# zju3dv/pats

Hardware: AMD Instinct MI355X
Metric: image-pairs/sec (coarse+fine OT) on 640x480 MegaDepth; OT iters/sec per pair (higher is better)
Workload: dtype f32 (contractions: fp32 operands split into fp16 hi + lo, three exact-product MFMA passes, fp32 accumulate)

## Files before the change

include/pats_amd.h:

```cpp
#ifndef PATS_AMD_H
#define PATS_AMD_H

#include <stddef.h>
#include <stdint.h>

#ifdef __cplusplus
extern "C" {
#endif

typedef void* pats_stream_t;

enum {
    PATS_OK = 0,
    PATS_ERR_INVALID = 1,
    PATS_ERR_UNSUPPORTED = 2,
    PATS_ERR_LAUNCH = 3,
    PATS_ERR_NO_DEVICE = 4
};

enum { PATS_SINKHORN_AUTO = 0, PATS_SINKHORN_LOG = 1, PATS_SINKHORN_KERNEL = 2 };

const char* pats_version(void);
#define PATS_ABI_VERSION 8
int pats_abi_version(void);
const char* pats_last_error(void);
int pats_device_count(void);
int pats_set_sinkhorn_mode(int mode);
int pats_set_fine_fused(int on);

int pats_sinkhorn_fallbacks(int64_t* count, int reset);

int pats_cost_f32(const float* d0, const float* d1, int64_t batch, int D, int n, int m, float* out,
                  pats_stream_t stream);

size_t pats_sinkhorn_workspace_bytes(int64_t batch, int M, int N);
int pats_sinkhorn_f32(const float* Z, int64_t batch, int M, int N, const float* log_mu,
                      const float* log_nu, int iters, float* out, void* workspace,
                      size_t workspace_bytes, pats_stream_t stream);

size_t pats_ot_workspace_bytes(int64_t batch, int M, int N);
int pats_log_optimal_transport_f32(const float* scores, int64_t batch, int m, int n,
                                   const float* alpha, const float* ns, int iters, float* Z,
                                   void* workspace, size_t workspace_bytes, pats_stream_t stream);

size_t pats_ot2_workspace_bytes(int64_t batch, int m, int n);
int pats_log_optimal_transport2_flags_f32(const float* scores, int64_t batch, int m, int n,
                                          const float* one, const float* ns, int iters, float bias_k,
                                          float* Z, uint8_t* col_nomatch, void* workspace,
                                          size_t workspace_bytes, pats_stream_t stream);
int pats_log_optimal_transport2_f32(const float* scores, int64_t batch, int m, int n,
                                    const float* one, const float* ns, int iters, float bias_k,
                                    float* Z, void* workspace, size_t workspace_bytes,
                                    pats_stream_t stream);

int pats_cost_ot_f32(const float* d0, const float* d1, int64_t batch, int D, int n, int m,
                     int variant, const float* scalar, const float* ns, int iters, float bias_k,
                     float* Z, void* workspace, size_t workspace_bytes, pats_stream_t stream);
size_t pats_cost_ot_workspace_bytes(int64_t batch, int D, int n, int m, int variant);
int pats_cost_ot_flags_f32(const float* d0, const float* d1, int64_t batch, int D, int n, int m,
                           int variant, const float* scalar, const float* ns, int iters, float bias_k,
                           float* Z, uint8_t* col_nomatch, void* workspace, size_t workspace_bytes,
                           pats_stream_t stream);

int pats_set_cost_ot_mid_event(void* event);

int pats_cost_ot_flags_counted_f32(const float* d0, const float* d1, int64_t batch_cap, const int64_t* batch_dev,
                                   int D, int n, int m, int variant, const float* scalar, const float* ns, int iters,
                                   float bias_k, float* Z, uint8_t* col_nomatch, void* workspace,
                                   size_t workspace_bytes, pats_stream_t stream);

int pats_colmass_sqrt_f32(const float* Z, int64_t batch, int M, int N, float* out,
                          pats_stream_t stream);
int pats_colmass_flags_f32(const float* Z, int64_t batch, int M, int N, float* out, uint8_t* col_nomatch,
                           pats_stream_t stream);
int pats_dustbin_bias_inplace_f32(float* Z, int64_t batch, int M, int N, float k,
                                  pats_stream_t stream);
int pats_exp_f32(const float* Z, int64_t count, float* out, pats_stream_t stream);

int pats_argmax_f32(const float* Z, int64_t batch, int M, int N, int64_t* row_arg,
                    int64_t* col_arg, pats_stream_t stream);

int pats_iterative_expand_f32(const float* P, int input_is_log, int64_t batch, int M, int N,
                              const float* scalex, const float* scaley, int lim3, int h, int w,
                              float lower_bound, int iter_num, float* whole_cost, float* core_cost,
                              float* average_point, float* x_scale, float* y_scale, int64_t* bound,
                              uint8_t* row_nomatch, pats_stream_t stream);

int pats_iterative_expand_counted_f32(const float* P, int input_is_log, int64_t batch_cap, const int64_t* batch_dev,
                                      int M, int N, const float* scalex, const float* scaley, int lim3, int h, int w,
                                      float lower_bound, int iter_num, float* whole_cost, float* core_cost,
                                      float* average_point, float* x_scale, float* y_scale, int64_t* bound,
                                      uint8_t* row_nomatch, pats_stream_t stream);

int pats_split_patches(const int32_t* sum_cycle_host, int height, int width, int max_once_used,
                       int64_t* second_layer_set, int64_t* third_layer_set);
int pats_split_patches_device(const int32_t* sum_cycle, int64_t pairs, int height, int width,
                              int max_once_used, int64_t* second_layer_set, int64_t* third_layer_set,
                              int32_t* cycle_num, pats_stream_t stream);

int pats_compute_imgs_bounds_f32(const float* x_scale, const float* y_scale,
                                 const float* average_point, const uint8_t* if_nomatching, int Np,
                                 int height, int width, int img, int64_t* bound5, int64_t* K_out,
                                 float* x_scale_new, float* y_scale_new, float* average_new,
                                 pats_stream_t stream);

int pats_left_crops_f32(const float* left, int n_img, int H, int W, const int64_t* bound5, int64_t K,
                        int height, int width, float* out, pats_stream_t stream);

int pats_compute_imgs_bounds_batch_f32(const float* x_scale, const float* y_scale, const float* average_point,
                                       const uint8_t* if_nomatching, int n_img, int Np, int height, int width,
                                       int64_t* bound5, int64_t* K_img, int64_t* K_total, float* x_scale_new,
// ... 266 lines not shown
```

pats_amd/_lib.py:

```python
import ctypes
import os

_HERE = os.path.dirname(os.path.abspath(__file__))
LIB_PATH = os.path.join(_HERE, "libpats_amd.so")
if os.environ.get("PATS_AMD_DIAG_LIB", "") not in ("", "0"):
    _sfx = os.environ["PATS_AMD_DIAG_LIB"]
    LIB_PATH = os.path.join(_HERE, "libpats_amd_diag%s.so" % ("" if _sfx == "1" else _sfx))

c_void_p, c_int, c_i64, c_f, c_size = (ctypes.c_void_p, ctypes.c_int, ctypes.c_int64, ctypes.c_float,
                                       ctypes.c_size_t)

ABI_VERSION = 8



class PairTable(ctypes.Structure):
    _fields_ = [("pairs", ctypes.c_int64), ("shape_host", c_void_p), ("cell_base_host", c_void_p), ("shape", c_void_p),
                ("cell_base", c_void_p), ("img_base", c_void_p)]


_TAB = ctypes.POINTER(PairTable)


class CropFormat(ctypes.Structure):
    _fields_ = [("dtype", ctypes.c_int32), ("layout", ctypes.c_int32), ("normalize", ctypes.c_int32),
                ("mean", ctypes.c_float * 3), ("std", ctypes.c_float * 3)]


_FMT = ctypes.POINTER(CropFormat)

SIGNATURES = {
    "pats_version": (ctypes.c_char_p, []),
    "pats_abi_version": (c_int, []),
    "pats_last_error": (ctypes.c_char_p, []),
    "pats_device_count": (c_int, []),
    "pats_set_sinkhorn_mode": (c_int, [c_int]),
    "pats_set_fine_fused": (c_int, [c_int]),
    "pats_sinkhorn_fallbacks": (c_int, [ctypes.POINTER(ctypes.c_int64), c_int]),
    "pats_set_gnn_redo_mode": (c_int, [c_int]),
    "pats_gnn_overflows": (c_int, [ctypes.POINTER(ctypes.c_int64), c_int]),
    "pats_cost_f32": (c_int, [c_void_p, c_void_p, c_i64, c_int, c_int, c_int, c_void_p, c_void_p]),
    "pats_sinkhorn_workspace_bytes": (c_size, [c_i64, c_int, c_int]),
    "pats_sinkhorn_f32": (c_int, [c_void_p, c_i64, c_int, c_int, c_void_p, c_void_p, c_int, c_void_p,
                                  c_void_p, c_size, c_void_p]),
    "pats_ot_workspace_bytes": (c_size, [c_i64, c_int, c_int]),
    "pats_log_optimal_transport_f32": (c_int, [c_void_p, c_i64, c_int, c_int, c_void_p, c_void_p, c_int,
                                               c_void_p, c_void_p, c_size, c_void_p]),
    "pats_ot2_workspace_bytes": (c_size, [c_i64, c_int, c_int]),
    "pats_log_optimal_transport2_f32": (c_int, [c_void_p, c_i64, c_int, c_int, c_void_p, c_void_p, c_int,
                                                c_f, c_void_p, c_void_p, c_size, c_void_p]),
    "pats_cost_ot_f32": (c_int, [c_void_p, c_void_p, c_i64, c_int, c_int, c_int, c_int, c_void_p,
                                 c_void_p, c_int, c_f, c_void_p, c_void_p, c_size, c_void_p]),
    "pats_cost_ot_flags_f32": (c_int, [c_void_p, c_void_p, c_i64, c_int, c_int, c_int, c_int, c_void_p,
                                       c_void_p, c_int, c_f, c_void_p, c_void_p, c_void_p, c_size, c_void_p]),
    "pats_set_cost_ot_mid_event": (c_int, [c_void_p]),
    "pats_cost_ot_flags_counted_f32": (c_int, [c_void_p, c_void_p, c_i64, c_void_p, c_int, c_int, c_int, c_int, c_void_p,
                                               c_void_p, c_int, c_f, c_void_p, c_void_p, c_void_p, c_size, c_void_p]),
    "pats_iterative_expand_counted_f32": (c_int, [c_void_p, c_int, c_i64, c_void_p, c_int, c_int, c_void_p, c_void_p, c_int,
                                                  c_int, c_int, c_f, c_int, c_void_p, c_void_p, c_void_p,
                                                  c_void_p, c_void_p, c_void_p, c_void_p, c_void_p]),
    "pats_fine_descriptors_counted_f32": (c_int, [c_void_p, c_void_p, c_void_p, c_void_p, c_void_p, c_i64, c_void_p, c_int,
                                                  c_void_p, c_void_p]),
    "pats_log_optimal_transport2_flags_f32": (c_int, [c_void_p, c_i64, c_int, c_int, c_void_p, c_void_p, c_int,
                                                      c_f, c_void_p, c_void_p, c_void_p, c_size, c_void_p]),
    "pats_colmass_flags_f32": (c_int, [c_void_p, c_i64, c_int, c_int, c_void_p, c_void_p, c_void_p]),
    "pats_cost_ot_workspace_bytes": (c_size, [c_i64, c_int, c_int, c_int, c_int]),
    "pats_colmass_sqrt_f32": (c_int, [c_void_p, c_i64, c_int, c_int, c_void_p, c_void_p]),
    "pats_dustbin_bias_inplace_f32": (c_int, [c_void_p, c_i64, c_int, c_int, c_f, c_void_p]),
    "pats_exp_f32": (c_int, [c_void_p, c_i64, c_void_p, c_void_p]),
    "pats_argmax_f32": (c_int, [c_void_p, c_i64, c_int, c_int, c_void_p, c_void_p, c_void_p]),
    "pats_iterative_expand_f32": (c_int, [c_void_p, c_int, c_i64, c_int, c_int, c_void_p, c_void_p, c_int,
                                          c_int, c_int, c_f, c_int, c_void_p, c_void_p, c_void_p,
                                          c_void_p, c_void_p, c_void_p, c_void_p, c_void_p]),
    "pats_split_patches": (c_int, [c_void_p, c_int, c_int, c_int, c_void_p, c_void_p]),
    "pats_split_patches_device": (c_int, [c_void_p, c_i64, c_int, c_int, c_int, c_void_p, c_void_p, c_void_p, c_void_p]),
    "pats_compute_imgs_bounds_batch_f32": (c_int, [c_void_p, c_void_p, c_void_p, c_void_p, c_int, c_int, c_int, c_int,
                                                   c_void_p, c_void_p, c_void_p, c_void_p, c_void_p, c_void_p, c_void_p]),
    "pats_left_crops_counted_f32": (c_int, [c_void_p, c_int, c_int, c_int, c_void_p, c_i64, c_void_p, c_int, c_int,
                                            c_void_p, c_void_p]),
    "pats_tensor_resize_hwc_counted_f32": (c_int, [c_void_p, c_int, c_int, c_int, c_int, c_void_p, c_i64, c_void_p,
                                                   c_void_p, c_void_p, c_void_p]),
    "pats_compute_imgs_bounds_f32": (c_int, [c_void_p, c_void_p, c_void_p, c_void_p, c_int, c_int, c_int,
                                             c_int, c_void_p, c_void_p, c_void_p, c_void_p, c_void_p,
                                             c_void_p]),
    "pats_left_crops_f32": (c_int, [c_void_p, c_int, c_int, c_int, c_void_p, c_i64, c_int, c_int, c_void_p,
                                    c_void_p]),
    "pats_tensor_resize_f32": (c_int, [c_void_p, c_int, c_int, c_int, c_int, c_void_p, c_i64, c_void_p,
                                       c_void_p, c_void_p]),
    "pats_tensor_resize_hwc_f32": (c_int, [c_void_p, c_int, c_int, c_int, c_int, c_void_p, c_i64,
                                           c_void_p, c_void_p, c_void_p]),
    "pats_compute_result_f32": (c_int, [c_void_p, c_int, c_i64, c_void_p, c_void_p, c_void_p, c_void_p,
                                        c_int, c_void_p, c_void_p, c_void_p, c_void_p, c_void_p,
                                        c_void_p]),
    "pats_compute_result_ws_f32": (c_int, [c_void_p, c_int, c_i64, c_void_p, c_void_p, c_void_p, c_void_p,
                                           c_int, c_void_p, c_void_p, c_void_p, c_void_p, c_void_p,
                                           c_void_p, c_size, c_void_p]),
    "pats_fine_descriptors_f32": (c_int, [c_void_p, c_void_p, c_void_p, c_void_p, c_void_p, c_i64, c_void_p, c_void_p]),
    "pats_third_descriptors_f32": (c_int, [c_void_p, c_void_p, c_void_p, c_void_p, c_void_p, c_void_p, c_void_p,
                                           c_i64, c_i64, c_void_p, c_void_p, c_void_p, c_void_p, c_void_p]),
    "pats_third_level_f32": (c_int, [c_void_p, c_void_p, c_i64, c_int, c_void_p, c_void_p, c_void_p, c_void_p,
                                     c_void_p, c_int, c_int, c_void_p, c_void_p, c_void_p, c_void_p, c_void_p,
                                     c_void_p]),
    "pats_third_descriptors_counted_f32": (c_int, [c_void_p, c_void_p, c_void_p, c_void_p, c_void_p, c_void_p, c_void_p,
                                                   c_i64, c_void_p, c_i64, c_void_p, c_void_p, c_void_p, c_void_p, c_void_p]),
    "pats_fine_descriptors_nhwc_f32": (c_int, [c_void_p, c_void_p, c_void_p, c_void_p, c_void_p, c_i64, c_void_p, c_void_p]),
    "pats_third_descriptors_nhwc_f32": (c_int, [c_void_p, c_void_p, c_void_p, c_void_p, c_void_p, c_void_p, c_void_p,
                                                c_i64, c_void_p, c_i64, c_void_p, c_void_p, c_void_p, c_void_p, c_void_p]),
    "pats_fine_descriptors_typed": (c_int, [c_void_p, c_void_p, c_void_p, c_int, c_int, c_void_p, c_void_p, c_i64, c_void_p,
                                            c_void_p, c_void_p]),
    "pats_third_descriptors_typed": (c_int, [c_void_p, c_void_p, c_int, c_int, c_void_p, c_void_p, c_void_p, c_void_p, c_void_p,
                                             c_i64, c_void_p, c_i64, c_void_p, c_void_p, c_void_p, c_void_p, c_void_p]),
    "pats_third_level_counted_f32": (c_int, [c_void_p, c_void_p, c_i64, c_void_p, c_int, c_void_p, c_void_p, c_void_p,
                                             c_void_p, c_void_p, c_int, c_int, c_void_p, c_void_p, c_void_p, c_void_p,
                                             c_void_p]),
    "pats_chunk_rows_workspace_bytes": (c_size, [c_i64, c_int]),
    "pats_chunk_rows_device": (c_int, [c_void_p, c_i64, c_int, c_int, c_int, c_int, c_i64] + [c_void_p] * 13 +
                               [c_size, c_void_p]),
    "pats_profile_marker": (c_int, [c_int, c_void_p]),
    "pats_stream_create_cu_mask": (c_int, [c_void_p, c_int, c_void_p]),
    "pats_stream_destroy": (c_int, [c_void_p]),
# ... 106 lines not shown
```

pats_amd/csrc/gather.hip:

```cpp
#include "common.hpp"

#include <cstdlib>

namespace pats {

template <int POL, typename T>
__device__ __forceinline__ T ldm(const T* p) {
    if (POL & 1) return __builtin_nontemporal_load(p);
    return *p;
}
template <int POL, typename T>
__device__ __forceinline__ void stm(T* p, T v) {
    if (POL & 2) __builtin_nontemporal_store(v, p);
    else *p = v;
}

typedef float f2u __attribute__((ext_vector_type(2), aligned(4)));
template <int POL>
__device__ __forceinline__ f2u ldm2(const float* p) {
    const f2u* q = reinterpret_cast<const f2u*>(p);
    if (POL & 1) return __builtin_nontemporal_load(q);
    return *q;
}

template <int POL>
__global__ void __launch_bounds__(256)
fine_desc_kernel(const float* __restrict__ f0, const float* __restrict__ f1,
                 const float* __restrict__ f2, const float* __restrict__ title,
                 const float* __restrict__ rubbish, int64_t B, float* __restrict__ desc,
                 const int64_t* __restrict__ B_live) {
    const int64_t n = blockIdx.x;
    const int64_t b = n % B;
    if (B_live && b >= *B_live) return;
    const int lane = threadIdx.x & 63, wave = threadIdx.x >> 6;
    float* o = desc + n * 264 * 145;
    int pt[3], off0[3], off1[3];
    bool live[3];
#pragma unroll
    for (int g = 0; g < 3; ++g) {
        const int p = lane + 64 * g;
        live[g] = p < 145;
        pt[g] = p < 144 ? p : 0;
        const int r = pt[g] / 12, c = pt[g] - r * 12;
        off0[g] = (4 * r + 1) * 48 + 4 * c + 1;
        off1[g] = (2 * r) * 24 + 2 * c;
    }
    const bool dust = lane == 16;
    auto put = [&](int ch, float v0, float v1, float v2) {
        float* row = o + ch * 145;
        stm<POL>(row + lane, v0);
        stm<POL>(row + lane + 64, v1);
        if (live[2]) stm<POL>(row + lane + 128, dust ? rubbish[b * 264 + ch] : v2);
    };
    for (int ch = wave; ch < 8; ch += 4) {
        const float v = title[b * 8 + ch];
        put(ch, v, v, v);
    }
#pragma unroll 2
    for (int ch = 8 + wave; ch < 72; ch += 4) {
        const float* m = f0 + (n * 64 + (ch - 8)) * 48 * 48;
        float v[3];
#pragma unroll
        for (int g = 0; g < 3; ++g) {
            const float* q = m + off0[g];
            const f2u a = ldm2<POL>(q), c2 = ldm2<POL>(q + 48);
            v[g] = (((a.x + a.y) + c2.x) + c2.y) / 4.0f;
        }
        put(ch, v[0], v[1], v[2]);
    }
#pragma unroll 2
    for (int ch = 72 + wave; ch < 136; ch += 4) {
        const float* m = f1 + (n * 64 + (ch - 72)) * 24 * 24;
        float v[3];
#pragma unroll
        for (int g = 0; g < 3; ++g) {
            const float* q = m + off1[g];
            const f2u a = ldm2<POL>(q), c2 = ldm2<POL>(q + 24);
            v[g] = (((a.x + a.y) + c2.x) + c2.y) / 4.0f;
        }
        put(ch, v[0], v[1], v[2]);
    }
#pragma unroll 4
    for (int ch = 136 + wave; ch < 264; ch += 4) {
        const float* m = f2 + (n * 128 + (ch - 136)) * 144;
        put(ch, ldm<POL>(m + pt[0]), ldm<POL>(m + pt[1]), ldm<POL>(m + pt[2]));
    }
}

__device__ __forceinline__ long long round_half_even_div(float x, float d) {
    return (long long)rintf(x / d);
}

template <int POL>
__global__ void __launch_bounds__(256)
third_desc_kernel(const float* __restrict__ ff0, const float* __restrict__ ff1,
                  const float* __restrict__ mk0, const float* __restrict__ mk1,
                  const int64_t* __restrict__ b_ids, const float* __restrict__ kenc,
                  const float* __restrict__ rubbish, int64_t P, int64_t B,
                  float* __restrict__ out0, float* __restrict__ out1, int64_t* __restrict__ ps_out,
                  int64_t* __restrict__ pt_out, const int64_t* __restrict__ P_dev) {
    constexpr int W = 8, M = 52, C = 128;
    int64_t live = P;
    if (P_dev) { const int64_t n = *P_dev; live = n < P ? n : P; }
    const int64_t per = (live + 7) >> 3, p = (int64_t)(blockIdx.x & 7) * per + (blockIdx.x >> 3);
    if ((int64_t)(blockIdx.x >> 3) >= per || p >= live) return;
    const int lane = threadIdx.x & 63, wave = threadIdx.x >> 6;
    const int64_t b = b_ids[p];
    const long long s0 = round_half_even_div(mk0[p * 2 + 0], 4.0f) * 4, s1 = round_half_even_div(mk0[p * 2 + 1], 4.0f) * 4;
    float t0 = mk1[p * 2 + 0], t1 = mk1[p * 2 + 1];
    t0 = t0 >= 96.f ? 96.f : t0; t1 = t1 >= 96.f ? 96.f : t1;
    t0 = t0 <= 0.f ? 0.f : t0;   t1 = t1 <= 0.f ? 0.f : t1;
    const long long q0 = round_half_even_div(t0, 4.0f) * 4, q1 = round_half_even_div(t1, 4.0f) * 4;
    if (threadIdx.x == 0) {
        if (ps_out) { ps_out[p * 2] = s0; ps_out[p * 2 + 1] = s1; }
        if (pt_out) { pt_out[p * 2] = q0; pt_out[p * 2 + 1] = q1; }
    }
    const int wx = lane % W, wy = lane / W;
    auto fdiv2 = [](long long v) { return v >= 0 ? v / 2 : -((-v + 1) / 2); };
    long long x0 = fdiv2(s0) + wx - W / 2 + 2, y0 = fdiv2(s1) + wy - W / 2 + 2;
    long long x1 = fdiv2(q0) + wx - W / 2 + 2, y1 = fdiv2(q1) + wy - W / 2 + 2;
    long long i0 = b * M * M + y0 * M + x0, i1 = b * M * M + y1 * M + x1;
    const long long lim = B * M * M - 1;
    i0 = i0 < 0 ? 0 : (i0 > lim ? lim : i0);
    i1 = i1 < 0 ? 0 : (i1 > lim ? lim : i1);
    long long x2 = round_half_even_div((float)s0, 8.0f), y2 = round_half_even_div((float)s1, 8.0f);
    long long i2 = b * 144 + y2 * 12 + x2;
    i2 = i2 < 0 ? 0 : (i2 > B * 144 - 1 ? B * 144 - 1 : i2);
    const long long bb2 = i2 / 144;
    i2 -= bb2 * 144;
    const long long bb0 = i0 / (M * M), r0 = i0 - bb0 * (M * M);
    const long long bb1 = i1 / (M * M), r1 = i1 - bb1 * (M * M);
    float* o0 = out0 + p * C * 65;
    float* o1 = out1 + p * C * 65;
    const float* src0 = ff0 + bb0 * C * (M * M) + r0;
    const float* src1 = ff1 + bb1 * C * (M * M) + r1;
#pragma unroll 1
    for (int c0 = 32 * wave; c0 < 32 * wave + 32; c0 += 8) {
        float a[8], c[8], ke[8];
#pragma unroll
        for (int k = 0; k < 8; ++k) {
            a[k] = ldm<POL>(src0 + (int64_t)(c0 + k) * (M * M));
            c[k] = ldm<POL>(src1 + (int64_t)(c0 + k) * (M * M));
            ke[k] = kenc[(c0 + k) * 64 + lane];
        }
#pragma unroll
        for (int k = 0; k < 8; ++k) {
            stm<POL>(o0 + (c0 + k) * 65 + lane, a[k] + ke[k]);
            stm<POL>(o1 + (c0 + k) * 65 + lane, c[k] + ke[k]);
        }
    }
    if (lane < 32) {
        const int ch = 32 * wave + lane;
        const float rb = rubbish[(bb2 * C + ch) * 144 + i2];
        o0[ch * 65 + 64] = rb;
        o1[ch * 65 + 64] = rb;
    }
}



template <int POL>
__global__ void __launch_bounds__(256)
third_desc_nhwc_kernel(const float* __restrict__ ff0, const float* __restrict__ ff1,
                       const float* __restrict__ mk0, const float* __restrict__ mk1,
                       const int64_t* __restrict__ b_ids, const float* __restrict__ kenc,
                       const float* __restrict__ rubbish, int64_t P, int64_t B,
                       float* __restrict__ out0, float* __restrict__ out1, int64_t* __restrict__ ps_out,
                       int64_t* __restrict__ pt_out, const int64_t* __restrict__ P_dev) {
    constexpr int W = 8, M = 52, C = 128, NT = 65;
    __shared__ __attribute__((aligned(16))) float tile[C * NT];
    int64_t live = P;
    if (P_dev) { const int64_t n = *P_dev; live = n < P ? n : P; }
    const unsigned k = blockIdx.x >> 3;
    const int side = k & 1;
    const int64_t per = (live + 7) >> 3, p = (int64_t)(blockIdx.x & 7) * per + (k >> 1);
    if ((int64_t)(k >> 1) >= per || p >= live) return;
    const int t = threadIdx.x, lane = t & 63, wave = __builtin_amdgcn_readfirstlane(t >> 6);
    const int64_t b = b_ids[p];
// ... 141 lines not shown
                      const uint16_t* __restrict__ f2, const float* __restrict__ title,
                      const float* __restrict__ rubbish, int64_t B, float* __restrict__ desc,
                      const int64_t* __restrict__ B_live) {
    const int64_t n = blockIdx.x;
    const int64_t b = n % B;
    if (B_live && b >= *B_live) return;
    const int lane = threadIdx.x & 63, wave = threadIdx.x >> 6;
    float* o = desc + n * 264 * 145;
    int pt[3], off0[3], off1[3];
    bool live[3];
#pragma unroll
    for (int g = 0; g < 3; ++g) {
        const int p = lane + 64 * g;
        live[g] = p < 145;
        pt[g] = p < 144 ? p : 0;
        const int r = pt[g] / 12, c = pt[g] - r * 12;
        off0[g] = (4 * r + 1) * 48 + 4 * c + 1;
        off1[g] = (2 * r) * 24 + 2 * c;
    }
    const bool dust = lane == 16;
    auto put = [&](int ch, float v0, float v1, float v2) {
        float* row = o + ch * 145;
        stm<POL>(row + lane, v0);
        stm<POL>(row + lane + 64, v1);
        if (live[2]) stm<POL>(row + lane + 128, dust ? rubbish[b * 264 + ch] : v2);
    };
    auto pool = [](uint32_t a, uint32_t c2) {
        return (((widen<DT>(a) + widen_hi<DT>(a)) + widen<DT>(c2)) + widen_hi<DT>(c2)) / 4.0f;
    };
    for (int ch = wave; ch < 8; ch += 4) {
        const float v = title[b * 8 + ch];
        put(ch, v, v, v);
    }
#pragma unroll 2
    for (int ch = 8 + wave; ch < 72; ch += 4) {
        const uint16_t* m = f0 + (n * 64 + (ch - 8)) * 48 * 48;
        float v[3];
#pragma unroll
        for (int g = 0; g < 3; ++g) v[g] = pool(ldh2<POL>(m + off0[g]), ldh2<POL>(m + off0[g] + 48));
        put(ch, v[0], v[1], v[2]);
    }
#pragma unroll 2
    for (int ch = 72 + wave; ch < 136; ch += 4) {
        const uint16_t* m = f1 + (n * 64 + (ch - 72)) * 24 * 24;
        float v[3];
#pragma unroll
        for (int g = 0; g < 3; ++g) v[g] = pool(ldh2<POL>(m + off1[g]), ldh2<POL>(m + off1[g] + 24));
        put(ch, v[0], v[1], v[2]);
    }
#pragma unroll 4
    for (int ch = 136 + wave; ch < 264; ch += 4) {
        const uint16_t* m = f2 + (n * 128 + (ch - 136)) * 144;
        put(ch, widen<DT>(ldm<POL>(m + pt[0])), widen<DT>(ldm<POL>(m + pt[1])), widen<DT>(ldm<POL>(m + pt[2])));
    }
}

struct third_point {
    long long i00[2], bb2, i2;
};
__device__ __forceinline__ third_point third_point_at(const float* __restrict__ mk0, const float* __restrict__ mk1,
                                                      int64_t p, int64_t b, int64_t B, bool write,
                                                      int64_t* __restrict__ ps_out, int64_t* __restrict__ pt_out) {
    constexpr int W = 8, M = 52;
    const long long s0 = round_half_even_div(mk0[p * 2 + 0], 4.0f) * 4, s1 = round_half_even_div(mk0[p * 2 + 1], 4.0f) * 4;
    float t0 = mk1[p * 2 + 0], t1 = mk1[p * 2 + 1];
    t0 = t0 >= 96.f ? 96.f : t0; t1 = t1 >= 96.f ? 96.f : t1;
    t0 = t0 <= 0.f ? 0.f : t0;   t1 = t1 <= 0.f ? 0.f : t1;
    const long long q0 = round_half_even_div(t0, 4.0f) * 4, q1 = round_half_even_div(t1, 4.0f) * 4;
    if (write) {
        if (ps_out) { ps_out[p * 2] = s0; ps_out[p * 2 + 1] = s1; }
        if (pt_out) { pt_out[p * 2] = q0; pt_out[p * 2 + 1] = q1; }
    }
    auto fdiv2 = [](long long v) { return v >= 0 ? v / 2 : -((-v + 1) / 2); };
    third_point r;
    r.i00[0] = b * M * M + (fdiv2(s1) - W / 2 + 2) * M + (fdiv2(s0) - W / 2 + 2);
    r.i00[1] = b * M * M + (fdiv2(q1) - W / 2 + 2) * M + (fdiv2(q0) - W / 2 + 2);
    long long i2 = b * 144 + round_half_even_div((float)s1, 8.0f) * 12 + round_half_even_div((float)s0, 8.0f);
    i2 = i2 < 0 ? 0 : (i2 > B * 144 - 1 ? B * 144 - 1 : i2);
    r.bb2 = i2 / 144;
    r.i2 = i2 - r.bb2 * 144;
    return r;
}

template <int DT, int POL>
__global__ void __launch_bounds__(256)
third_desc_half_kernel(const uint16_t* __restrict__ ff0, const uint16_t* __restrict__ ff1,
                       const float* __restrict__ mk0, const float* __restrict__ mk1,
                       const int64_t* __restrict__ b_ids, const float* __restrict__ kenc,
                       const float* __restrict__ rubbish, int64_t P, int64_t B,
                       float* __restrict__ out0, float* __restrict__ out1, int64_t* __restrict__ ps_out,
                       int64_t* __restrict__ pt_out, const int64_t* __restrict__ P_dev) {
    constexpr int M = 52, C = 128;
    int64_t live = P;
    if (P_dev) { const int64_t n = *P_dev; live = n < P ? n : P; }
    const int64_t per = (live + 7) >> 3, p = (int64_t)(blockIdx.x & 7) * per + (blockIdx.x >> 3);
    if ((int64_t)(blockIdx.x >> 3) >= per || p >= live) return;
    const int lane = threadIdx.x & 63, wave = threadIdx.x >> 6;
    const int cp = lane & 31, sub = lane >> 5;
    const int64_t b = b_ids[p];
    const third_point tp = third_point_at(mk0, mk1, p, b, B, threadIdx.x == 0, ps_out, pt_out);
    const long long lim = B * M * M - 1;
    const uint16_t* src[2];
    bool below[2], above[2];
#pragma unroll
    for (int s = 0; s < 2; ++s) {
        const long long i = tp.i00[s] + (cp >> 2) * M + 2 * (cp & 3);
        below[s] = i < 0;
        above[s] = i > lim;
        const long long j = below[s] ? 0 : (above[s] ? lim - 1 : i);
        const long long bb = j / (M * M);
        src[s] = (s ? ff1 : ff0) + bb * C * (M * M) + (j - bb * (M * M));
    }
    auto fix = [](uint32_t u, bool lo, bool hi) {
        u = lo ? (u & 0xffffu) * 0x10001u : u;
        return hi ? (u >> 16) * 0x10001u : u;
    };
    float* o0 = out0 + p * C * 65 + 2 * cp;
    float* o1 = out1 + p * C * 65 + 2 * cp;
#pragma unroll 1
    for (int c0 = 32 * wave + sub; c0 < 32 * wave + 32; c0 += 16) {
        uint32_t a[8], c[8];
        f2s ke[8];
#pragma unroll
        for (int k = 0; k < 8; ++k) {
            a[k] = ldm<POL>(reinterpret_cast<const uint32_t*>(src[0] + (int64_t)(c0 + 2 * k) * (M * M)));
            c[k] = ldm<POL>(reinterpret_cast<const uint32_t*>(src[1] + (int64_t)(c0 + 2 * k) * (M * M)));
            ke[k] = *reinterpret_cast<const f2s*>(kenc + (c0 + 2 * k) * 64 + 2 * cp);
        }
#pragma unroll
        for (int k = 0; k < 8; ++k) {
            const uint32_t u = fix(a[k], below[0], above[0]), v = fix(c[k], below[1], above[1]);
            f2s x, y;
            x.x = widen<DT>(u) + ke[k].x; x.y = widen_hi<DT>(u) + ke[k].y;
            y.x = widen<DT>(v) + ke[k].x; y.y = widen_hi<DT>(v) + ke[k].y;
            stm2<POL>(o0 + (c0 + 2 * k) * 65, x);
            stm2<POL>(o1 + (c0 + 2 * k) * 65, y);
        }
    }
    if (lane < 32) {
        const int ch = 32 * wave + lane;
        const float rb = rubbish[(tp.bb2 * C + ch) * 144 + tp.i2];
        out0[p * C * 65 + ch * 65 + 64] = rb;
        out1[p * C * 65 + ch * 65 + 64] = rb;
    }
}

template <int DT, int POL>
__global__ void __launch_bounds__(256)
third_desc_nhwc_half_kernel(const uint16_t* __restrict__ ff0, const uint16_t* __restrict__ ff1,
                            const float* __restrict__ mk0, const float* __restrict__ mk1,
                            const int64_t* __restrict__ b_ids, const float* __restrict__ kenc,
                            const float* __restrict__ rubbish, int64_t P, int64_t B,
                            float* __restrict__ out0, float* __restrict__ out1, int64_t* __restrict__ ps_out,
                            int64_t* __restrict__ pt_out, const int64_t* __restrict__ P_dev) {
    constexpr int M = 52, C = 128, NT = 65;
    __shared__ __attribute__((aligned(16))) float tile[C * NT];
    int64_t live = P;
    if (P_dev) { const int64_t n = *P_dev; live = n < P ? n : P; }
    const unsigned k = blockIdx.x >> 3;
    const int side = k & 1;
    const int64_t per = (live + 7) >> 3, p = (int64_t)(blockIdx.x & 7) * per + (k >> 1);
    if ((int64_t)(k >> 1) >= per || p >= live) return;
    const int t = threadIdx.x, lane = t & 63, wave = __builtin_amdgcn_readfirstlane(t >> 6);
    const int64_t b = b_ids[p];
    const third_point tp = third_point_at(mk0, mk1, p, b, B, t == 0 && side == 0, ps_out, pt_out);
    const long long lim = B * M * M - 1;
// ... 47 lines not shown
#pragma unroll
    for (int g = 0; g < 5; ++g) {
        const int nd = 32 * g + 8 * wave + sub, r = nd / 12, c = nd - 12 * r;
        if (g < 4 || wave < 2) {
            const uint16_t* px = img + ((step * r + first) * rowpix + step * c + first) * cpp + ch0 + 8 * cg;
#pragma unroll
            for (int tap = 0; tap < TAPS; ++tap)
                q[g][tap] = ldm<POL>(reinterpret_cast<const u4*>(px + ((tap >> 1) * rowpix + (tap & 1)) * cpp));
        }
    }
#pragma unroll
    for (int g = 0; g < 5; ++g) {
        const int nd = 32 * g + 8 * wave + sub;
        if (g < 4 || wave < 2) {
#pragma unroll
            for (int h = 0; h < 8; ++h) {
                float v;
                if (TAPS == 4) {
                    float x[4];
#pragma unroll
                    for (int tap = 0; tap < 4; ++tap) x[tap] = h & 1 ? widen_hi<DT>(q[g][tap][h >> 1]) : widen<DT>(q[g][tap][h >> 1]);
                    v = (((x[0] + x[1]) + x[2]) + x[3]) / 4.0f;
                } else {
                    v = h & 1 ? widen_hi<DT>(q[g][0][h >> 1]) : widen<DT>(q[g][0][h >> 1]);
                }
                tile[(8 * cg + h) * NP + nd] = v;
            }
        }
    }
    if (t < 64) tile[t * NP + 144] = dust;
    wg_barrier();
    const f4* src = reinterpret_cast<const f4*>(tile);
    f4* dst = reinterpret_cast<f4*>(o);
    for (int e = t; e < 64 * NP / 4; e += 256) stm<POL>(dst + e, src[e]);
    wg_barrier();
}

template <int DT, int POL>
__global__ void __launch_bounds__(256)
fine_desc_nhwc_half_kernel(const uint16_t* __restrict__ f0, const uint16_t* __restrict__ f1,
                           const uint16_t* __restrict__ f2, const float* __restrict__ title,
                           const float* __restrict__ rubbish, int64_t B, float* __restrict__ desc,
                           const int64_t* __restrict__ B_live) {
    constexpr int NP = 145;
    __shared__ __attribute__((aligned(16))) float tile[64 * NP];
    const int64_t n = blockIdx.x;
    const int64_t b = n % B;
    if (B_live && b >= *B_live) return;
    const int t = threadIdx.x;
    float* o = desc + n * 264 * NP;
    const float* rub = rubbish + b * 264;
    for (int e = t; e < 8 * NP; e += 256) {
        const int ch = e / NP, p = e - ch * NP;
        o[e] = p == 144 ? rub[ch] : title[b * 8 + ch];
    }
    fine_tile_pass_half<DT, 4, POL>(f0 + n * 48 * 48 * 64, 64, 0, 48, 4, 1, tile, o + 8 * NP, rub + 8, t);
    fine_tile_pass_half<DT, 4, POL>(f1 + n * 24 * 24 * 64, 64, 0, 24, 2, 0, tile, o + 72 * NP, rub + 72, t);
    fine_tile_pass_half<DT, 1, POL>(f2 + n * 144 * 128, 128, 0, 12, 1, 0, tile, o + 136 * NP, rub + 136, t);
    fine_tile_pass_half<DT, 1, POL>(f2 + n * 144 * 128, 128, 64, 12, 1, 0, tile, o + 200 * NP, rub + 200, t);
}

static int gather_policy(bool channels_last) {
    static const int pol = [] { const char* e = env_switch("PATS_GATHER_NT"); return e ? (atoi(e) & 3) : -1; }();
    return pol >= 0 ? pol : (channels_last ? 3 : 0);
}
#define GATHER_LAUNCH(KERNEL, NHWC, grid, ...)                                                                                \
    switch (gather_policy(NHWC)) {                                                                                           \
        case 0: hipLaunchKernelGGL((KERNEL<0>), grid, dim3(256), 0, as_stream(stream), __VA_ARGS__); break;                  \
        case 1: hipLaunchKernelGGL((KERNEL<1>), grid, dim3(256), 0, as_stream(stream), __VA_ARGS__); break;                  \
        case 2: hipLaunchKernelGGL((KERNEL<2>), grid, dim3(256), 0, as_stream(stream), __VA_ARGS__); break;                  \
        default: hipLaunchKernelGGL((KERNEL<3>), grid, dim3(256), 0, as_stream(stream), __VA_ARGS__); break;                 \
    }
#define GATHER_LAUNCH_HALF(KERNEL, DT, NHWC, grid, ...)                                                                       \
    switch (gather_policy(NHWC)) {                                                                                           \
        case 0: hipLaunchKernelGGL((KERNEL<DT, 0>), grid, dim3(256), 0, as_stream(stream), __VA_ARGS__); break;              \
        case 1: hipLaunchKernelGGL((KERNEL<DT, 1>), grid, dim3(256), 0, as_stream(stream), __VA_ARGS__); break;              \
        case 2: hipLaunchKernelGGL((KERNEL<DT, 2>), grid, dim3(256), 0, as_stream(stream), __VA_ARGS__); break;              \
        default: hipLaunchKernelGGL((KERNEL<DT, 3>), grid, dim3(256), 0, as_stream(stream), __VA_ARGS__); break;             \
    }
#define GATHER_LAUNCH_TYPED(KERNEL, DTYPE, NHWC, grid, ...)                                                                   \
    if ((DTYPE) == PATS_MAP_F16) { GATHER_LAUNCH_HALF(KERNEL, PATS_MAP_F16, NHWC, grid, __VA_ARGS__) }                        \
    else { GATHER_LAUNCH_HALF(KERNEL, PATS_MAP_BF16, NHWC, grid, __VA_ARGS__) }

}

using namespace pats;

extern "C" int pats_fine_descriptors_f32(const float* feat0, const float* feat1, const float* feat2,
                                         const float* title, const float* rubbish, int64_t B,
                                         float* desc, pats_stream_t stream) {
    PATS_REQUIRE(B >= 0, "fine_descriptors: bad shape");
    if (B == 0) return PATS_OK;
    PATS_REQUIRE(feat0 && feat1 && feat2 && title && rubbish && desc, "fine_descriptors: null pointer");
    GATHER_LAUNCH(fine_desc_kernel, false, dim3((unsigned)(2 * B)), feat0, feat1,
                       feat2, title, rubbish, B, desc, (const int64_t*)nullptr);
    return check_launch("fine_desc_kernel");
}

extern "C" int pats_fine_descriptors_counted_f32(const float* feat0, const float* feat1, const float* feat2,
                                                 const float* title, const float* rubbish, int64_t B_cap,
                                                 const int64_t* B_dev, int channels_last, float* desc, pats_stream_t stream) {
    PATS_REQUIRE(B_cap >= 0, "fine_descriptors_counted: bad shape");
    if (B_cap == 0) return PATS_OK;
    PATS_REQUIRE(B_dev && feat0 && feat1 && feat2 && title && rubbish && desc, "fine_descriptors_counted: null pointer");
    if (channels_last) {
        PATS_REQUIRE(((uintptr_t)feat0 | (uintptr_t)feat1 | (uintptr_t)feat2 | (uintptr_t)desc) % 16 == 0,
                     "fine_descriptors_counted: channels-last maps and desc must be 16-byte aligned");
        GATHER_LAUNCH(fine_desc_nhwc_kernel, true, dim3((unsigned)(2 * B_cap)), feat0, feat1,
                           feat2, title, rubbish, B_cap, desc, B_dev);
        return check_launch("fine_desc_nhwc_kernel");
    }
    GATHER_LAUNCH(fine_desc_kernel, false, dim3((unsigned)(2 * B_cap)), feat0, feat1,
                       feat2, title, rubbish, B_cap, desc, B_dev);
    return check_launch("fine_desc_kernel");
}

extern "C" int pats_third_descriptors_f32(const float* feat_f0, const float* feat_f1,
                                          const float* mkpts0_c, const float* mkpts1_c,
                                          const int64_t* b_ids, const float* kenc, const float* rubbish,
                                          int64_t P, int64_t B, float* out0, float* out1,
                                          int64_t* p_s_out, int64_t* p_t_out, pats_stream_t stream) {
    PATS_REQUIRE(P >= 0 && B > 0, "third_descriptors: bad shape");
    if (P == 0) return PATS_OK;
    PATS_REQUIRE(feat_f0 && feat_f1 && mkpts0_c && mkpts1_c && b_ids && kenc && rubbish && out0 && out1,
                 "third_descriptors: null pointer");
    GATHER_LAUNCH(third_desc_kernel, false, dim3((unsigned)((P + 7) / 8 * 8)), feat_f0, feat_f1,
                       mkpts0_c, mkpts1_c, b_ids, kenc, rubbish, P, B, out0, out1, p_s_out, p_t_out, (const int64_t*)nullptr);
    return check_launch("third_desc_kernel");
}

extern "C" int pats_third_descriptors_counted_f32(const float* feat_f0, const float* feat_f1,
                                                  const float* mkpts0_c, const float* mkpts1_c,
                                                  const int64_t* b_ids, const float* kenc, const float* rubbish,
                                                  int64_t P_cap, const int64_t* P_dev, int64_t B, float* out0, float* out1,
                                                  int64_t* p_s_out, int64_t* p_t_out, pats_stream_t stream) {
    PATS_REQUIRE(P_cap >= 0 && B > 0, "third_descriptors_counted: bad shape");
    if (P_cap == 0) return PATS_OK;
    PATS_REQUIRE(P_dev && feat_f0 && feat_f1 && mkpts0_c && mkpts1_c && b_ids && kenc && rubbish && out0 && out1,
                 "third_descriptors_counted: null pointer");
    GATHER_LAUNCH(third_desc_kernel, false, dim3((unsigned)((P_cap + 7) / 8 * 8)), feat_f0, feat_f1,
                       mkpts0_c, mkpts1_c, b_ids, kenc, rubbish, P_cap, B, out0, out1, p_s_out, p_t_out, P_dev);
    return check_launch("third_desc_kernel");
}

extern "C" int pats_fine_descriptors_nhwc_f32(const float* feat0, const float* feat1, const float* feat2,
                                              const float* title, const float* rubbish, int64_t B,
                                              float* desc, pats_stream_t stream) {
    PATS_REQUIRE(B >= 0, "fine_descriptors_nhwc: bad shape");
    if (B == 0) return PATS_OK;
    PATS_REQUIRE(feat0 && feat1 && feat2 && title && rubbish && desc, "fine_descriptors_nhwc: null pointer");
    PATS_REQUIRE(((uintptr_t)feat0 | (uintptr_t)feat1 | (uintptr_t)feat2 | (uintptr_t)desc) % 16 == 0,
                 "fine_descriptors_nhwc: maps and desc must be 16-byte aligned");
    GATHER_LAUNCH(fine_desc_nhwc_kernel, true, dim3((unsigned)(2 * B)), feat0, feat1,
                       feat2, title, rubbish, B, desc, (const int64_t*)nullptr);
    return check_launch("fine_desc_nhwc_kernel");
}

extern "C" int pats_third_descriptors_nhwc_f32(const float* feat_f0, const float* feat_f1,
                                               const float* mkpts0_c, const float* mkpts1_c,
                                               const int64_t* b_ids, const float* kenc, const float* rubbish,
                                               int64_t P_cap, const int64_t* P_dev, int64_t B, float* out0, float* out1,
                                               int64_t* p_s_out, int64_t* p_t_out, pats_stream_t stream) {
    PATS_REQUIRE(P_cap >= 0 && B > 0, "third_descriptors_nhwc: bad shape");
    if (P_cap == 0) return PATS_OK;
    PATS_REQUIRE(feat_f0 && feat_f1 && mkpts0_c && mkpts1_c && b_ids && kenc && rubbish && out0 && out1,
                 "third_descriptors_nhwc: null pointer");
    GATHER_LAUNCH(third_desc_nhwc_kernel, true, dim3((unsigned)((P_cap + 7) / 8 * 16)), feat_f0,
                       feat_f1, mkpts0_c, mkpts1_c, b_ids, kenc, rubbish, P_cap, B, out0, out1, p_s_out, p_t_out, P_dev);
    return check_launch("third_desc_nhwc_kernel");
}


extern "C" int pats_fine_descriptors_typed(const void* feat0, const void* feat1, const void* feat2, pats_map_dtype_t dtype,
                                           int channels_last, const float* title, const float* rubbish, int64_t B_cap,
                                           const int64_t* B_dev, float* desc, pats_stream_t stream) {
    PATS_REQUIRE(dtype == PATS_MAP_F32 || dtype == PATS_MAP_F16 || dtype == PATS_MAP_BF16,
                 "fine_descriptors_typed: unknown map dtype %d", (int)dtype);
    PATS_REQUIRE(B_cap >= 0, "fine_descriptors_typed: bad shape");
    if (B_cap == 0) return PATS_OK;
    PATS_REQUIRE(feat0 && feat1 && feat2 && title && rubbish && desc, "fine_descriptors_typed: null pointer");
    const uintptr_t maps = (uintptr_t)feat0 | (uintptr_t)feat1 | (uintptr_t)feat2;
    if (channels_last)
        PATS_REQUIRE((maps | (uintptr_t)desc) % 16 == 0, "fine_descriptors_typed: channels-last maps and desc must be 16-byte aligned");
    else
        PATS_REQUIRE(maps % 4 == 0, "fine_descriptors_typed: NCHW maps must be 4-byte aligned");
    const dim3 grid((unsigned)(2 * B_cap));
    if (dtype == PATS_MAP_F32) {
        const float *f0 = (const float*)feat0, *f1 = (const float*)feat1, *f2 = (const float*)feat2;
        if (channels_last) {
            GATHER_LAUNCH(fine_desc_nhwc_kernel, true, grid, f0, f1, f2, title, rubbish, B_cap, desc, B_dev);
            return check_launch("fine_desc_nhwc_kernel");
        }
        GATHER_LAUNCH(fine_desc_kernel, false, grid, f0, f1, f2, title, rubbish, B_cap, desc, B_dev);
        return check_launch("fine_desc_kernel");
    }
    const uint16_t *h0 = (const uint16_t*)feat0, *h1 = (const uint16_t*)feat1, *h2 = (const uint16_t*)feat2;
    if (channels_last) {
        GATHER_LAUNCH_TYPED(fine_desc_nhwc_half_kernel, dtype, true, grid, h0, h1, h2, title, rubbish, B_cap, desc, B_dev);
        return check_launch("fine_desc_nhwc_half_kernel");
    }
    GATHER_LAUNCH_TYPED(fine_desc_half_kernel, dtype, false, grid, h0, h1, h2, title, rubbish, B_cap, desc, B_dev);
    return check_launch("fine_desc_half_kernel");
}

extern "C" int pats_third_descriptors_typed(const void* feat_f0, const void* feat_f1, pats_map_dtype_t dtype, int channels_last,
                                            const float* mkpts0_c, const float* mkpts1_c, const int64_t* b_ids,
                                            const float* kenc, const float* rubbish, int64_t P_cap, const int64_t* P_dev,
                                            int64_t B, float* out0, float* out1, int64_t* p_s_out, int64_t* p_t_out,
                                            pats_stream_t stream) {
    PATS_REQUIRE(dtype == PATS_MAP_F32 || dtype == PATS_MAP_F16 || dtype == PATS_MAP_BF16,
                 "third_descriptors_typed: unknown map dtype %d", (int)dtype);
    PATS_REQUIRE(P_cap >= 0 && B > 0, "third_descriptors_typed: bad shape");
    if (P_cap == 0) return PATS_OK;
    PATS_REQUIRE(feat_f0 && feat_f1 && mkpts0_c && mkpts1_c && b_ids && kenc && rubbish && out0 && out1,
                 "third_descriptors_typed: null pointer");
    const uintptr_t maps = (uintptr_t)feat_f0 | (uintptr_t)feat_f1;
    if (channels_last)
        PATS_REQUIRE(maps % (dtype == PATS_MAP_F32 ? 4 : 16) == 0, "third_descriptors_typed: channels-last maps must be %d-byte aligned",
                     dtype == PATS_MAP_F32 ? 4 : 16);
    else
        PATS_REQUIRE(maps % 4 == 0, "third_descriptors_typed: NCHW maps must be 4-byte aligned");
    if (dtype == PATS_MAP_F32) {
        const float *f0 = (const float*)feat_f0, *f1 = (const float*)feat_f1;
        if (channels_last) {
            GATHER_LAUNCH(third_desc_nhwc_kernel, true, dim3((unsigned)((P_cap + 7) / 8 * 16)), f0, f1, mkpts0_c, mkpts1_c, b_ids,
                          kenc, rubbish, P_cap, B, out0, out1, p_s_out, p_t_out, P_dev);
            return check_launch("third_desc_nhwc_kernel");
        }
        GATHER_LAUNCH(third_desc_kernel, false, dim3((unsigned)((P_cap + 7) / 8 * 8)), f0, f1, mkpts0_c, mkpts1_c, b_ids,
                      kenc, rubbish, P_cap, B, out0, out1, p_s_out, p_t_out, P_dev);
        return check_launch("third_desc_kernel");
    }
    const uint16_t *h0 = (const uint16_t*)feat_f0, *h1 = (const uint16_t*)feat_f1;
    if (channels_last) {
        GATHER_LAUNCH_TYPED(third_desc_nhwc_half_kernel, dtype, true, dim3((unsigned)((P_cap + 7) / 8 * 16)), h0, h1, mkpts0_c,
                            mkpts1_c, b_ids, kenc, rubbish, P_cap, B, out0, out1, p_s_out, p_t_out, P_dev);
        return check_launch("third_desc_nhwc_half_kernel");
    }
    GATHER_LAUNCH_TYPED(third_desc_half_kernel, dtype, false, dim3((unsigned)((P_cap + 7) / 8 * 8)), h0, h1, mkpts0_c, mkpts1_c,
                        b_ids, kenc, rubbish, P_cap, B, out0, out1, p_s_out, p_t_out, P_dev);
    return check_launch("third_desc_half_kernel");
}
```

pats_amd/ops.py:

```python
import ctypes

import numpy as np
import torch

from . import _lib

_L = _lib.lib
_check = _lib.check
_L()


_raw_stream = getattr(torch._C, "_cuda_getCurrentRawStream", None)


def _stream():
    if _raw_stream is not None:
        return ctypes.c_void_p(_raw_stream(torch.cuda.current_device()))
    return ctypes.c_void_p(torch.cuda.current_stream().cuda_stream)


def _dev(t, name, dtype=torch.float32):
    if not isinstance(t, torch.Tensor):
        raise TypeError("%s must be a torch.Tensor" % name)
    if not t.is_cuda:
# ... 4 lines not shown
    return t.contiguous()


def _map(t, name, dtype=torch.float32):
    if not isinstance(t, torch.Tensor):
        raise TypeError("%s must be a torch.Tensor" % name)
    if not t.is_cuda:
        raise RuntimeError("pats_amd: %s is on %s; the HIP path needs a GPU tensor (no CPU fallback)" % (name, t.device))
    if t.dtype != dtype:
        raise RuntimeError("pats_amd: %s must be %s, got %s" % (name, dtype, t.dtype))
    if t.dim() == 4 and not t.is_contiguous() and t.is_contiguous(memory_format=torch.channels_last):
        return t, True
    return t.contiguous(), False


_MAP_DTYPES = {torch.float32: 0, torch.float16: 1, torch.bfloat16: 2}


def _maps_any(tensors, names):
    for t, name in zip(tensors, names):
        if not isinstance(t, torch.Tensor):
            raise TypeError("%s must be a torch.Tensor" % name)
        if t.dtype not in _MAP_DTYPES:
            raise RuntimeError("pats_amd: %s must be float32, float16 or bfloat16, got %s" % (name, t.dtype))
    dtypes = {t.dtype for t in tensors}
    if dtypes == {torch.float32}:
        return [_map(t, n) for t, n in zip(tensors, names)], None
    if len(dtypes) != 1:
        return [_map(t.float(), n) for t, n in zip(tensors, names)], None
    dt = tensors[0].dtype
    maps = [_map(t, n, dt) for t, n in zip(tensors, names)]
    if len({cl for _, cl in maps}) != 1:
        maps = [(t.contiguous(), False) for t, _ in maps]
    align = 16 if maps[0][1] else 4
    if any(t.data_ptr() % align for t, _ in maps):
        return [_map(t.float(), n) for t, n in zip(tensors, names)], None
    return maps, _MAP_DTYPES[dt]


def _ptr(t):
    return ctypes.c_void_p(t.data_ptr()) if t is not None else ctypes.c_void_p(0)


_WS = {}
_WS_MAX = 64 << 20
_WS_ON = [False]


class workspace_cache:

    def __enter__(self):
        self.prev = _WS_ON[0]
        _WS_ON[0] = True

    def __exit__(self, *exc):
        _WS_ON[0] = self.prev


def _workspace(nbytes, device):
    n = max(int(nbytes), 1)
    if not _WS_ON[0] or n > _WS_MAX or _raw_stream is None or torch.cuda.is_current_stream_capturing():
        return torch.empty(n, dtype=torch.uint8, device=device)
    key = (device.index, _raw_stream(torch.cuda.current_device()))
    t = _WS.get(key)
    if t is None or t.numel() < n:
        t = _WS[key] = torch.empty(min(_WS_MAX, max(2 * n, 1 << 20)), dtype=torch.uint8, device=device)
    return t


def _scalar_dev(x, device):
    if isinstance(x, torch.Tensor):
        return x.detach().reshape(1).to(device=device, dtype=torch.float32)
    return torch.full((1,), float(x), dtype=torch.float32, device=device)


def set_sinkhorn_mode(mode):
    names = {"auto": 0, "log": 1, "kernel": 2}
    prev = _L().pats_set_sinkhorn_mode(names[mode])
    return {v: k for k, v in names.items()}[prev]


def set_fine_fused(on):
    return bool(_L().pats_set_fine_fused(1 if on else 0))


def sinkhorn_fallbacks(reset=True):
    import ctypes
    n = ctypes.c_int64(0)
    rc = _L().pats_sinkhorn_fallbacks(ctypes.byref(n), 1 if reset else 0)
    if rc != 0:
        raise RuntimeError(_L().pats_last_error().decode())
    return int(n.value)


def set_gnn_redo(mode):
    names = {"inline": 0, "deferred": 1}
    prev = _L().pats_set_gnn_redo_mode(names[mode])
    return {v: k for k, v in names.items()}[prev]


def gnn_overflows(reset=True):
    n = ctypes.c_int64(0)
    _check(_L().pats_gnn_overflows(ctypes.byref(n), 1 if reset else 0), "gnn_overflows")
    return bool(n.value)


def cost(mdesc0, mdesc1, out=None):
    d0, d1 = _dev(mdesc0, "mdesc0"), _dev(mdesc1, "mdesc1")
    b, D, n = d0.shape
    if d1.shape[0] != b or d1.shape[1] != D:
        raise RuntimeError("cost: descriptor shapes %s / %s do not match" % (tuple(d0.shape), tuple(d1.shape)))
    m = d1.shape[2]
    if out is None:
        out = torch.empty((b, n, m), dtype=torch.float32, device=d0.device)
    elif tuple(out.shape) != (b, n, m) or out.dtype != torch.float32 or not out.is_contiguous() or out.device != d0.device:
        raise RuntimeError("cost: out must be a contiguous float32 [%d, %d, %d] tensor on %s" % (b, n, m, d0.device))
    _check(_L().pats_cost_f32(_ptr(d0), _ptr(d1), b, D, n, m, _ptr(out), _stream()), "cost")
    return out


def log_sinkhorn_iterations(Z, log_mu, log_nu, iters: int):
    Z, log_mu, log_nu = _dev(Z, "Z"), _dev(log_mu, "log_mu"), _dev(log_nu, "log_nu")
    b, M, N = Z.shape
    if tuple(log_mu.shape) != (b, M) or tuple(log_nu.shape) != (b, N):
        raise RuntimeError("log_sinkhorn_iterations: marginal shapes do not match Z")
    out = torch.empty_like(Z)
    nb = _L().pats_sinkhorn_workspace_bytes(b, M, N)
    ws = _workspace(nb, Z.device)
    _check(_L().pats_sinkhorn_f32(_ptr(Z), b, M, N, _ptr(log_mu), _ptr(log_nu), int(iters), _ptr(out),
                                  _ptr(ws), nb, _stream()), "log_sinkhorn_iterations")
    return out


def log_optimal_transport(scores, alpha, ns, iters: int):
    scores = _dev(scores, "scores")
    b, m, n = scores.shape
    ns = _dev(ns, "ns")
    if ns.numel() != b * n:
        raise RuntimeError("log_optimal_transport: ns must have %d entries per batch" % n)
    ns = ns.reshape(b, n)
    a = _scalar_dev(alpha, scores.device)
    Z = torch.empty((b, m + 1, n + 1), dtype=torch.float32, device=scores.device)
    nb = _L().pats_ot_workspace_bytes(b, m + 1, n + 1)
    ws = _workspace(nb, scores.device)
    _check(_L().pats_log_optimal_transport_f32(_ptr(scores), b, m, n, _ptr(a), _ptr(ns), int(iters),
                                               _ptr(Z), _ptr(ws), nb, _stream()), "log_optimal_transport")
    return Z


def log_optimal_transport2(scores, one, ns, iters: int, bias_k: float = 0.0):
    scores = _dev(scores, "scores")
    b, m, n = scores.shape
    ns = _dev(ns, "ns")
    if ns.numel() != b * (n - 1):
        raise RuntimeError("log_optimal_transport2: ns must have %d entries per batch" % (n - 1))
    ns = ns.reshape(b, n - 1)
    o = _scalar_dev(one, scores.device)
    Z = torch.empty((b, m, n), dtype=torch.float32, device=scores.device)
    nb = _L().pats_ot2_workspace_bytes(b, m, n)
    ws = _workspace(nb, scores.device)
    _check(_L().pats_log_optimal_transport2_f32(_ptr(scores), b, m, n, _ptr(o), _ptr(ns), int(iters),
                                                float(bias_k), _ptr(Z), _ptr(ws), nb, _stream()),
           "log_optimal_transport2")
    return Z


# ... 1405 lines not shown
```

Measured before the change: 1868.

## Add tiled third-stage descriptor gather with LDS-staged vectorized stores

Adds a new NCHW f32 third-descriptor kernel. Each wave handles two points, gathers 8 channels at a time, and stages them in LDS so the output rows can be written as contiguous 16-byte vector stores rather than scattered scalar writes. The old per-point kernel is kept and selected when the mode setter asks for it or when the outputs are not 16-byte aligned; the tiled path is the default. The aim is better store coalescing and fewer blocks, in exchange for LDS use and extra wave syncs.

New measurement: 1932 (median of 6 runs). 1.03x the previous value.

```diff
diff --git a/include/pats_amd.h b/include/pats_amd.h
--- a/include/pats_amd.h
+++ b/include/pats_amd.h
@@ -27,6 +27,8 @@
 int pats_device_count(void);
 int pats_set_sinkhorn_mode(int mode);
 int pats_set_fine_fused(int on);
+
+int pats_set_third_gather(int mode);
 
 int pats_sinkhorn_fallbacks(int64_t* count, int reset);
 
diff --git a/pats_amd/_lib.py b/pats_amd/_lib.py
--- a/pats_amd/_lib.py
+++ b/pats_amd/_lib.py
@@ -36,6 +36,7 @@
     "pats_device_count": (c_int, []),
     "pats_set_sinkhorn_mode": (c_int, [c_int]),
     "pats_set_fine_fused": (c_int, [c_int]),
+    "pats_set_third_gather": (c_int, [c_int]),
     "pats_sinkhorn_fallbacks": (c_int, [ctypes.POINTER(ctypes.c_int64), c_int]),
     "pats_set_gnn_redo_mode": (c_int, [c_int]),
     "pats_gnn_overflows": (c_int, [ctypes.POINTER(ctypes.c_int64), c_int]),
diff --git a/pats_amd/csrc/gather.hip b/pats_amd/csrc/gather.hip
--- a/pats_amd/csrc/gather.hip
+++ b/pats_amd/csrc/gather.hip
@@ -93,7 +93,7 @@
 
 template <int POL>
 __global__ void __launch_bounds__(256)
-third_desc_kernel(const float* __restrict__ ff0, const float* __restrict__ ff1,
+third_desc_point_kernel(const float* __restrict__ ff0, const float* __restrict__ ff1,
                   const float* __restrict__ mk0, const float* __restrict__ mk1,
                   const int64_t* __restrict__ b_ids, const float* __restrict__ kenc,
                   const float* __restrict__ rubbish, int64_t P, int64_t B,
@@ -401,6 +401,83 @@
     return r;
 }
 
+constexpr int THIRD_TILE = 8;
+
+template <int POL>
+__global__ void __launch_bounds__(256)
+third_desc_kernel(const float* __restrict__ ff0, const float* __restrict__ ff1,
+                  const float* __restrict__ mk0, const float* __restrict__ mk1,
+                  const int64_t* __restrict__ b_ids, const float* __restrict__ kenc,
+                  const float* __restrict__ rubbish, int64_t P, int64_t B,
+                  float* __restrict__ out0, float* __restrict__ out1, int64_t* __restrict__ ps_out,
+                  int64_t* __restrict__ pt_out, const int64_t* __restrict__ P_dev) {
+    constexpr int PW = THIRD_TILE / 4;
+    constexpr int M = 52, C = 128, NT = 65, T = THIRD_TILE, SPAN = 8 * NT;
+    typedef float f4 __attribute__((ext_vector_type(4)));
+    __shared__ __attribute__((aligned(16))) float stage[4 * PW * SPAN];
+    int64_t live = P;
+    if (P_dev) { const int64_t n = *P_dev; live = n < P ? n : P; }
+    const int64_t tiles = (live + T - 1) / T, per = (tiles + 7) >> 3, tile = (int64_t)(blockIdx.x & 7) * per + (blockIdx.x >> 3);
+    if ((int64_t)(blockIdx.x >> 3) >= per || tile >= tiles) return;
+    const int lane = threadIdx.x & 63, wave = __builtin_amdgcn_readfirstlane(threadIdx.x >> 6);
+    const long long lim = B * M * M - 1;
+    int64_t pp[PW];
+    bool on[PW];
+    const float* src[PW][2];
+    const float* rub[PW];
+#pragma unroll
+    for (int j = 0; j < PW; ++j) {
+        const int64_t p = tile * T + wave * PW + j;
+        on[j] = p < live;
+        pp[j] = on[j] ? p : live - 1;
+        const int64_t b = b_ids[pp[j]];
+        const third_point tp = third_point_at(mk0, mk1, pp[j], b, B, on[j] && lane == 0, ps_out, pt_out);
+#pragma unroll
+        for (int s = 0; s < 2; ++s) {
+            long long i = tp.i00[s] + (lane >> 3) * M + (lane & 7);
+            i = i < 0 ? 0 : (i > lim ? lim : i);
+            const long long bb = i / (M * M);
+            src[j][s] = (s ? ff1 : ff0) + bb * C * (M * M) + (i - bb * (M * M));
+        }
+        rub[j] = rubbish + tp.bb2 * C * 144 + tp.i2;
+    }
+    float* slice = stage + wave * PW * SPAN;
+#pragma unroll 1
+    for (int c0 = 0; c0 < C; c0 += 8) {
+        float a[PW][2][8], ke[8], rb[PW];
+#pragma unroll
+        for (int k = 0; k < 8; ++k) {
+#pragma unroll
+            for (int j = 0; j < PW; ++j) {
+                a[j][0][k] = ldm<POL>(src[j][0] + (int64_t)(c0 + k) * (M * M));
+                a[j][1][k] = ldm<POL>(src[j][1] + (int64_t)(c0 + k) * (M * M));
+            }
+            ke[k] = kenc[(c0 + k) * 64 + lane];
+        }
+#pragma unroll
+        for (int j = 0; j < PW; ++j) rb[j] = lane < 8 ? rub[j][(c0 + lane) * 144] : 0.f;
+#pragma unroll
+        for (int j = 0; j < PW; ++j) {
+            float* sl = slice + j * SPAN;
+#pragma unroll
+            for (int s = 0; s < 2; ++s) {
+#pragma unroll
+                for (int k = 0; k < 8; ++k) sl[k * NT + lane] = a[j][s][k] + ke[k];
+                if (lane < 8) sl[lane * NT + 64] = rb[j];
+                wave_lds_sync();
+                const f4* v = reinterpret_cast<const f4*>(sl);
+                f4* o = reinterpret_cast<f4*>((s ? out1 : out0) + pp[j] * (C * NT) + c0 * NT);
+                if (on[j]) {
+                    stm<POL>(o + lane, v[lane]);
+                    stm<POL>(o + lane + 64, v[lane + 64]);
+                    if (lane < SPAN / 4 - 128) stm<POL>(o + lane + 128, v[lane + 128]);
+                }
+                wave_lds_sync();
+            }
+        }
+    }
+}
+
 template <int DT, int POL>
 __global__ void __launch_bounds__(256)
 third_desc_half_kernel(const uint16_t* __restrict__ ff0, const uint16_t* __restrict__ ff1,
@@ -614,9 +691,30 @@
     if ((DTYPE) == PATS_MAP_F16) { GATHER_LAUNCH_HALF(KERNEL, PATS_MAP_F16, NHWC, grid, __VA_ARGS__) }                        \
     else { GATHER_LAUNCH_HALF(KERNEL, PATS_MAP_BF16, NHWC, grid, __VA_ARGS__) }
 
+static int g_third_gather = 0;
+static int launch_third_nchw_f32(const float* f0, const float* f1, const float* mkpts0_c, const float* mkpts1_c,
+                                 const int64_t* b_ids, const float* kenc, const float* rubbish, int64_t P_cap, const int64_t* P_dev,
+                                 int64_t B, float* out0, float* out1, int64_t* p_s_out, int64_t* p_t_out, pats_stream_t stream) {
+    if (g_third_gather == 1 || ((uintptr_t)out0 | (uintptr_t)out1) % 16 != 0) {
+        GATHER_LAUNCH(third_desc_point_kernel, false, dim3((unsigned)((P_cap + 7) / 8 * 8)), f0, f1, mkpts0_c, mkpts1_c, b_ids,
+                      kenc, rubbish, P_cap, B, out0, out1, p_s_out, p_t_out, P_dev);
+        return check_launch("third_desc_point_kernel");
+    }
+    const int64_t tiles = (P_cap + THIRD_TILE - 1) / THIRD_TILE;
+    GATHER_LAUNCH(third_desc_kernel, false, dim3((unsigned)((tiles + 7) / 8 * 8)), f0, f1, mkpts0_c, mkpts1_c, b_ids, kenc, rubbish,
+                  P_cap, B, out0, out1, p_s_out, p_t_out, P_dev);
+    return check_launch("third_desc_kernel");
+}
+
 }
 
 using namespace pats;
+
+extern "C" int pats_set_third_gather(int mode) {
+    const int prev = g_third_gather;
+    if (mode == 0 || mode == 1) g_third_gather = mode;
+    return prev;
+}
 
 extern "C" int pats_fine_descriptors_f32(const float* feat0, const float* feat1, const float* feat2,
                                          const float* title, const float* rubbish, int64_t B,
@@ -656,9 +754,8 @@
     if (P == 0) return PATS_OK;
     PATS_REQUIRE(feat_f0 && feat_f1 && mkpts0_c && mkpts1_c && b_ids && kenc && rubbish && out0 && out1,
                  "third_descriptors: null pointer");
-    GATHER_LAUNCH(third_desc_kernel, false, dim3((unsigned)((P + 7) / 8 * 8)), feat_f0, feat_f1,
-                       mkpts0_c, mkpts1_c, b_ids, kenc, rubbish, P, B, out0, out1, p_s_out, p_t_out, (const int64_t*)nullptr);
-    return check_launch("third_desc_kernel");
+    return launch_third_nchw_f32(feat_f0, feat_f1, mkpts0_c, mkpts1_c, b_ids, kenc, rubbish, P, nullptr, B, out0, out1, p_s_out,
+                                 p_t_out, stream);
 }
 
 extern "C" int pats_third_descriptors_counted_f32(const float* feat_f0, const float* feat_f1,
@@ -670,9 +767,8 @@
     if (P_cap == 0) return PATS_OK;
     PATS_REQUIRE(P_dev && feat_f0 && feat_f1 && mkpts0_c && mkpts1_c && b_ids && kenc && rubbish && out0 && out1,
                  "third_descriptors_counted: null pointer");
-    GATHER_LAUNCH(third_desc_kernel, false, dim3((unsigned)((P_cap + 7) / 8 * 8)), feat_f0, feat_f1,
-                       mkpts0_c, mkpts1_c, b_ids, kenc, rubbish, P_cap, B, out0, out1, p_s_out, p_t_out, P_dev);
-    return check_launch("third_desc_kernel");
+    return launch_third_nchw_f32(feat_f0, feat_f1, mkpts0_c, mkpts1_c, b_ids, kenc, rubbish, P_cap, P_dev, B, out0, out1, p_s_out,
+                                 p_t_out, stream);
 }
 
 extern "C" int pats_fine_descriptors_nhwc_f32(const float* feat0, const float* feat1, const float* feat2,
@@ -759,9 +855,8 @@
                           kenc, rubbish, P_cap, B, out0, out1, p_s_out, p_t_out, P_dev);
             return check_launch("third_desc_nhwc_kernel");
         }
-        GATHER_LAUNCH(third_desc_kernel, false, dim3((unsigned)((P_cap + 7) / 8 * 8)), f0, f1, mkpts0_c, mkpts1_c, b_ids,
-                      kenc, rubbish, P_cap, B, out0, out1, p_s_out, p_t_out, P_dev);
-        return check_launch("third_desc_kernel");
+        return launch_third_nchw_f32(f0, f1, mkpts0_c, mkpts1_c, b_ids, kenc, rubbish, P_cap, P_dev, B, out0, out1, p_s_out,
+                                     p_t_out, stream);
     }
     const uint16_t *h0 = (const uint16_t*)feat_f0, *h1 = (const uint16_t*)feat_f1;
     if (channels_last) {
diff --git a/pats_amd/ops.py b/pats_amd/ops.py
--- a/pats_amd/ops.py
+++ b/pats_amd/ops.py
@@ -110,6 +110,14 @@
 
 def set_fine_fused(on):
     return bool(_L().pats_set_fine_fused(1 if on else 0))
+
+
+def set_third_gather(mode):
+    modes = {"tile": 0, "point": 1}
+    if mode not in modes:
+        raise ValueError("set_third_gather: mode must be 'tile' or 'point'")
+    prev = _L().pats_set_third_gather(modes[mode])
+    return {v: k for k, v in modes.items()}.get(prev, "tile")
 
 
 def sinkhorn_fallbacks(reset=True):
```
